# djene-mengistu/UAPS

Hardware: AMD Instinct MI355X
Metric: training images/sec (labeled+unlabeled) NEU-Seg 256x256 K=3 (higher is better)
Workload: dtype f32

## Files before the change

### uaps_amd/csrc/conv_split_wrw.hpp

```cpp
#pragma once
#include "conv_split.hpp"

namespace uaps {

#ifndef UAPS_WRW_ABLATE
#define UAPS_WRW_ABLATE 0
#endif

template <int TH, int WCO, int WCI, int DIL = 1> struct SWrwCfg {
    static constexpr int TW = 32, WR = 4 / (WCO * WCI), RPW = TH / WR;
    static constexpr int BCO = 16 * WCO, BCI = 16 * WCI;
    static constexpr int XG = DIL > 1 ? 6 : 4;
    static constexpr int DPLU = TH * 4 + 2;
    static constexpr int XPLU = (TH + 2) * XG + 2;
    static constexpr int EPL = (TH + 2) * 4 + 1;
    static constexpr int ND = (BCO * TH * 4 + kConvThreads - 1) / kConvThreads;
    static constexpr int NX = (BCI * (TH + 2) * XG + kConvThreads - 1) / kConvThreads;
    static_assert(WCO * WCI * WR == 4 && TH % WR == 0, "wave arrangement");
};

__device__ __forceinline__ void split8(const float (&v)[8], u32x4& p0, u32x4& p1, u32x4& p2) {
#pragma unroll
    for (int i = 0; i < 4; ++i) {
        unsigned a, b, c;
        conv_split3(v[2 * i], v[2 * i + 1], a, b, c);
        p0[i] = a; p1[i] = b; p2[i] = c;
    }
}

__device__ __forceinline__ void split8h(const float (&v)[8], float sc, u32x4& p0, u32x4& p1) {
    const f32x2 sc2 = bcast_lo(sc);
#pragma unroll
    for (int i = 0; i < 4; ++i) {
        const f32x2 t = f32x2{v[2 * i], v[2 * i + 1]} * sc2;
        unsigned a, b;
        conv_split2h(t.x, t.y, a, b);
        p0[i] = a; p1[i] = b;
    }
}

template <int TH, int WCO, int WCI, bool XF, bool H16 = false, int DIL = 1>
__device__ __forceinline__ void conv_swrw_body(const ConvWrwArgs& a) {
    using Cfg = SWrwCfg<TH, WCO, WCI, DIL>;
    static_assert(DIL == 1 || ((DIL == 2 || DIL == 4) && H16 && !XF), "dilated form: fp16 pieces, no staging-time BatchNorm");
    constexpr int NP = H16 ? 2 : 3;
    constexpr int XG = Cfg::XG, XH = DIL > 1 ? 1 : 0;
    constexpr int TW = 32, WR = Cfg::WR, RPW = Cfg::RPW, BCO = Cfg::BCO, BCI = Cfg::BCI;
    constexpr int DPLU = Cfg::DPLU, XPLU = Cfg::XPLU, EPL = Cfg::EPL, ND = Cfg::ND, NX = Cfg::NX;
    constexpr int RED_FLOATS = WR > 1 ? (WR / 2) * WCO * WCI * 10 * 256 : 0;
    constexpr bool EU = H16 && DIL == 1;
    constexpr int XGS = EU ? 5 : XG;
    constexpr int XPLS = EU ? (TH + 2) * 5 + ((TH + 2) * 5 % 4 == 2 ? 0 : (6 - (TH + 2) * 5 % 4) % 4) : XPLU;
    static_assert(XPLS % 4 == 2, "input plane stride");
    constexpr int NE = EU ? (BCI * (TH + 2) + kConvThreads - 1) / kConvThreads : 0;
    constexpr int STAGE_UNITS = NP * BCO * DPLU + NP * BCI * XPLS;
    constexpr int LDS_UNITS = STAGE_UNITS > RED_FLOATS / 4 ? STAGE_UNITS : RED_FLOATS / 4;

    __shared__ __attribute__((aligned(16))) u32x4 smem[LDS_UNITS];
    __shared__ unsigned sE[(DIL == 1 && !EU) ? NP * BCI * EPL : 1];
    __shared__ f32x2 sXf[XF ? kWrwMaxGroups * BCI + 1 : 1];
    u32x4* sD = smem;
    u32x4* sX = smem + NP * BCO * DPLU;
    constexpr int XF_ZERO = kWrwMaxGroups * BCI;

    float sc_d = 1.f, sc_x = 1.f, inv_d = 1.f, inv_x = 1.f;
    if constexpr (H16) {
        const f32x2 sd = h16_scale(bound_of(a.dy_bound, a.dy_mul));
        const f32x2 sx = h16_scale(__builtin_fmaxf(bound_of(a.in_bound, a.in_mul), bound_of(a.in2_bound, a.in2_mul)));
        sc_d = sd.x; inv_d = sd.y; sc_x = sx.x; inv_x = sx.y;
    }

    const int tid = threadIdx.x, lane = tid & 63, wave = tid >> 6;
    const int j = lane & 15, kq = lane >> 4;
    const int wr = wave % WR, wci = (wave / WR) % WCI, wco = wave / (WR * WCI);

    int bid = xcd_swizzle(blockIdx.x, gridDim.x);
    if (bid >= a.nsplit * a.ncob * a.ncib) return;
    stagger_by_wave_slot();
    const int cib = bid % a.ncib; bid /= a.ncib;
    const int cob = bid % a.ncob;
    const int split = bid / a.ncob;
    const int co0 = cob * BCO, ci0 = cib * BCI;
    const int HW = a.H * a.W;
    const int tiles_per_img = a.tiles_x * a.tiles_y, ntiles = a.B * tiles_per_img;
    const int t_begin = (int)((long)ntiles * split / a.nsplit), t_end = (int)((long)ntiles * (split + 1) / a.nsplit);
    const bool want_bias = a.bslab != nullptr && cib == 0;

    int dC[ND], dR[ND], dG[ND];
    int xC[NX], xR[NX], xG[NX];
#pragma unroll
    for (int n = 0; n < ND; ++n) {
        const int u = tid + n * kConvThreads;
        dC[n] = u < BCO * TH * 4 ? u / (TH * 4) : -1; dR[n] = (u / 4) % TH; dG[n] = u % 4;
    }
#pragma unroll
    for (int n = 0; n < NX; ++n) {
        const int u = tid + n * kConvThreads;
        xC[n] = u < BCI * (TH + 2) * XG ? u / ((TH + 2) * XG) : -1; xR[n] = (u / XG) % (TH + 2); xG[n] = u % XG;
    }
    if constexpr (XF) {
        const int G = a.B / a.xf_Bg;
        for (int i = tid; i < G * BCI; i += kConvThreads) {
            const int g = i / BCI, ch = ci0 + i % BCI;
            f32x2 v = f32x2{0.f, 0.f};
            if (ch < a.Cin) { const float2 t = a.xf[(size_t)g * a.Cin + ch]; v = f32x2{t.x, t.y}; }
            sXf[i] = v;
        }
        if (tid == 0) sXf[XF_ZERO] = f32x2{0.f, 0.f};
    }

    float rd[ND][8];
    float rx[NX][(DIL == 1 && !EU) ? 10 : 8];
    float re[EU ? NE : 1][2];
    int eC[EU ? NE : 1], eR[EU ? NE : 1];
    if constexpr (EU) {
#pragma unroll
        for (int n = 0; n < NE; ++n) {
            const int i = tid + n * kConvThreads;
            eC[n] = i < BCI * (TH + 2) ? i / (TH + 2) : -1; eR[n] = i % (TH + 2);
        }
    }
    int xf_idx[XF ? NX : 1];
    int exf_idx[(XF && EU) ? NE : 1];

    auto load_tile = [&](int t) {
        const int b = t / tiles_per_img, tt = t % tiles_per_img;
        const int ry = a.col_major ? tt % a.tiles_y : tt / a.tiles_x, x0 = (a.col_major ? tt / a.tiles_y : tt % a.tiles_x) * TW;
        const int y0 = DIL == 1 ? ry * TH : ry % DIL + (ry / DIL) * (TH * DIL);
#pragma unroll
        for (int n = 0; n < ND; ++n) {
            const int c = co0 + dC[n], gy = y0 + dR[n] * DIL, gx = x0 + dG[n] * 8;
#if UAPS_WRW_ABLATE & 4
            {
                const int cc = c < 0 ? 0 : (c < a.Cout ? c : a.Cout - 1), yy = gy < a.H ? gy : a.H - 1, xx = gx + 8 <= a.W ? gx : a.W - 8;
                const float* q = a.dout + ((size_t)b * a.Cout + cc) * HW + yy * a.W + xx;
                const f32x4 w0 = *reinterpret_cast<const f32x4*>(q), w1 = *reinterpret_cast<const f32x4*>(q + 4);
#pragma unroll
                for (int k = 0; k < 4; ++k) { rd[n][k] = w0[k]; rd[n][4 + k] = w1[k]; }
                continue;
            }
#endif
            const bool ok = dC[n] >= 0 && c < a.Cout && gy < a.H && gx < a.W;
            const float* p = a.dout + ((size_t)b * a.Cout + (ok ? c : 0)) * HW + (ok ? gy * a.W + gx : 0);
            const f32x4 v0 = ok ? *reinterpret_cast<const f32x4*>(p) : f32x4{0.f, 0.f, 0.f, 0.f};
            const f32x4 v1 = (ok && gx + 4 < a.W) ? *reinterpret_cast<const f32x4*>(p + 4) : f32x4{0.f, 0.f, 0.f, 0.f};
#pragma unroll
            for (int k = 0; k < 4; ++k) { rd[n][k] = v0[k]; rd[n][4 + k] = v1[k]; }
        }
#pragma unroll
        for (int n = 0; n < NX; ++n) {
            const int c = ci0 + xC[n], gy = y0 + (xR[n] - 1) * DIL, gx = x0 + (xG[n] - XH) * 8;
#if UAPS_WRW_ABLATE & 8
            if (xR[n] == 0 || xR[n] == TH + 1) continue;
#endif
#if UAPS_WRW_ABLATE & 4
            {
                const int cc = c < 0 ? 0 : (c < a.Csplit ? c : a.Csplit - 1), yy = gy < 0 ? 0 : (gy < a.H ? gy : a.H - 1);
                const int xx = gx < 0 ? 0 : (gx + 8 <= a.W ? gx : a.W - 8);
                const float* q = a.in + ((size_t)b * a.Csplit + cc) * HW + yy * a.W;
                const f32x4 w0 = *reinterpret_cast<const f32x4*>(q + xx), w1 = *reinterpret_cast<const f32x4*>(q + xx + 4);
#pragma unroll
                for (int k = 0; k < 4; ++k) { rx[n][k] = w0[k]; rx[n][4 + k] = w1[k]; }
                if constexpr (DIL == 1 && !EU) {
#if !(UAPS_WRW_ABLATE & 2)
                    rx[n][8] = q[xx > 0 ? xx - 1 : 0]; rx[n][9] = q[xx + 8 < a.W ? xx + 8 : a.W - 1];
#else
                    rx[n][8] = 0.f; rx[n][9] = 0.f;
#endif
                }
                if constexpr (XF) xf_idx[n] = (b / a.xf_Bg) * BCI + (xC[n] < 0 ? 0 : xC[n]);
                continue;
            }
#endif
            const bool second = c >= a.Csplit;
            const float* src = second ? a.in2 + ((size_t)b * (a.Cin - a.Csplit) + (c - a.Csplit)) * HW : a.in + ((size_t)b * a.Csplit + c) * HW;
            const bool okc = xC[n] >= 0 && c < a.Cin && gy >= 0 && gy < a.H;
            const bool ok = okc && gx >= 0 && gx < a.W;
            const float* p = src + (okc ? gy * a.W : 0) + (ok ? gx : 0);
            const f32x4 v0 = ok ? *reinterpret_cast<const f32x4*>(p) : f32x4{0.f, 0.f, 0.f, 0.f};
            const f32x4 v1 = (ok && gx + 4 < a.W) ? *reinterpret_cast<const f32x4*>(p + 4) : f32x4{0.f, 0.f, 0.f, 0.f};
#pragma unroll
            for (int k = 0; k < 4; ++k) { rx[n][k] = v0[k]; rx[n][4 + k] = v1[k]; }
            if constexpr (DIL == 1 && !EU) {
#if UAPS_WRW_ABLATE & 2
                rx[n][8] = 0.f; rx[n][9] = 0.f;
#else
                rx[n][8] = (okc && gx - 1 >= 0 && gx - 1 < a.W) ? src[gy * a.W + gx - 1] : 0.f;
                rx[n][9] = (okc && gx + 8 < a.W) ? src[gy * a.W + gx + 8] : 0.f;
#endif
            }
            if constexpr (XF) xf_idx[n] = okc ? (b / a.xf_Bg) * BCI + xC[n] : XF_ZERO;
        }
        if constexpr (EU) {
#pragma unroll
            for (int n = 0; n < NE; ++n) {
                const int c = ci0 + eC[n], gy = y0 + eR[n] - 1;
                const bool second = c >= a.Csplit;
                const float* src = second ? a.in2 + ((size_t)b * (a.Cin - a.Csplit) + (c - a.Csplit)) * HW : a.in + ((size_t)b * a.Csplit + c) * HW;
                const bool okc = eC[n] >= 0 && c < a.Cin && gy >= 0 && gy < a.H;
#if UAPS_WRW_ABLATE & 2
                re[n][0] = 0.f; re[n][1] = 0.f;
#else
                re[n][0] = (okc && x0 - 1 >= 0) ? src[gy * a.W + x0 - 1] : 0.f;
                re[n][1] = (okc && x0 + TW < a.W) ? src[gy * a.W + x0 + TW] : 0.f;
#endif
                if constexpr (XF) exf_idx[n] = okc ? (b / a.xf_Bg) * BCI + eC[n] : XF_ZERO;
            }
        }
    };
    auto store_tile = [&](int t) {
        const int tt = t % tiles_per_img;
        const int x0 = (a.col_major ? tt / a.tiles_y : tt % a.tiles_x) * TW;
#pragma unroll
        for (int n = 0; n < ND; ++n) {
            if (dC[n] < 0) continue;
            const int u = dC[n] * DPLU + dR[n] * 4 + dG[n];
            if constexpr (H16) {
                u32x4 p0, p1;
                split8h(rd[n], sc_d, p0, p1);
                sD[u] = p0; sD[BCO * DPLU + u] = p1;
            } else {
                u32x4 p0, p1, p2;
                split8(rd[n], p0, p1, p2);
                sD[u] = p0; sD[BCO * DPLU + u] = p1; sD[2 * BCO * DPLU + u] = p2;
            }
        }
#pragma unroll
        for (int n = 0; n < NX; ++n) {
            if (xC[n] < 0) continue;
#if UAPS_WRW_ABLATE & 8
            if (xR[n] == 0 || xR[n] == TH + 1) continue;
#endif
            if constexpr (XF) {
                const f32x2 cf = sXf[xf_idx[n]];
                const int gx = x0 + xG[n] * 8;
#pragma unroll
                for (int k = 0; k < ((DIL == 1 && !EU) ? 10 : 8); ++k) {
                    const int col = k < 8 ? gx + k : (k == 8 ? gx - 1 : gx + 8);
                    const float z = __builtin_fmaf(rx[n][k], cf.x, cf.y);
                    rx[n][k] = (col >= 0 && col < a.W) ? __builtin_fmaxf(z, z * a.xf_slope) : 0.f;
                }
            }
            float v8[8];
#pragma unroll
            for (int k = 0; k < 8; ++k) v8[k] = rx[n][k];
            const int u = xC[n] * XPLS + xR[n] * XGS + xG[n];
            const int eu = xC[n] * EPL + xR[n] * 4 + xG[n];
            if constexpr (DIL > 1) {
                u32x4 p0, p1;
                split8h(v8, sc_x, p0, p1);
                sX[u] = p0; sX[BCI * XPLS + u] = p1;
            } else if constexpr (EU) {
                u32x4 p0, p1;
                split8h(v8, sc_x, p0, p1);
                sX[u] = p0; sX[BCI * XPLS + u] = p1;
                (void)eu;
            } else if constexpr (H16) {
                u32x4 p0, p1;
                split8h(v8, sc_x, p0, p1);
                sX[u] = p0; sX[BCI * XPLS + u] = p1;
#if !(UAPS_WRW_ABLATE & 2)
                unsigned e0, e1;
                const f32x2 ev = f32x2{rx[n][9], rx[n][8]} * bcast_lo(sc_x);
                conv_split2h(ev.x, ev.y, e0, e1);
                sE[eu] = e0; sE[BCI * EPL + eu] = e1;
#else
                (void)eu;
#endif
            } else {
                u32x4 p0, p1, p2;
                split8(v8, p0, p1, p2);
                sX[u] = p0; sX[BCI * XPLS + u] = p1; sX[2 * BCI * XPLS + u] = p2;
                unsigned e0, e1, e2;
                conv_split3(rx[n][9], rx[n][8], e0, e1, e2);
                sE[eu] = e0; sE[BCI * EPL + eu] = e1; sE[2 * BCI * EPL + eu] = e2;
            }
        }
        if constexpr (EU) {
#if !(UAPS_WRW_ABLATE & 2)
#pragma unroll
            for (int n = 0; n < NE; ++n) {
                if (eC[n] < 0) continue;
                float l = re[n][0], r = re[n][1];
                if constexpr (XF) {
                    const f32x2 cf = sXf[exf_idx[n]];
                    const float zl = __builtin_fmaf(l, cf.x, cf.y), zr = __builtin_fmaf(r, cf.x, cf.y);
                    l = x0 - 1 >= 0 ? __builtin_fmaxf(zl, zl * a.xf_slope) : 0.f;
                    r = x0 + TW < a.W ? __builtin_fmaxf(zr, zr * a.xf_slope) : 0.f;
                }
                unsigned e0, e1;
                const f32x2 ev = f32x2{r, l} * bcast_lo(sc_x);
                conv_split2h(ev.x, ev.y, e0, e1);
                const int ue = eC[n] * XPLS + eR[n] * XGS + 4;
                sX[ue] = u32x4{e0, e0, e0, e0}; sX[BCI * XPLS + ue] = u32x4{e1, e1, e1, e1};
            }
#endif
        }
    };

    f32x4 acc[9];
    f32x4 accb = f32x4{0.f, 0.f, 0.f, 0.f};
#pragma unroll
    for (int t = 0; t < 9; ++t) acc[t] = f32x4{0.f, 0.f, 0.f, 0.f};
    constexpr unsigned kOnes = H16 ? 0x3C003C00u : 0x3F803F80u;
    const u32x4 ones_u = u32x4{kOnes, kOnes, kOnes, kOnes};
    const bf16x8 ones = __builtin_bit_cast(bf16x8, ones_u);

    const int aoff = (wco * 16 + j) * DPLU + kq;
    const int boff = (wci * 16 + j) * XPLS + kq + XH;
    const int eoff = (wci * 16 + j) * EPL + kq;
    const int elidx = ((kq + 4) % 5) * 4 + 3, eridx = (kq + 1) * 4;

    if (t_begin < t_end) { load_tile(t_begin); }
    if constexpr (XF) __syncthreads();
    if (t_begin < t_end) store_tile(t_begin);
    __syncthreads();
    for (int t = t_begin; t < t_end; ++t) {
        const bool more = t + 1 < t_end;
        if (more) load_tile(t + 1);
#pragma unroll
        for (int rr = 0; rr < RPW + 2; ++rr) {
            const int r = wr * RPW + rr;
            bf16x8 bf[3][NP];
#pragma unroll
            for (int p = 0; p < NP; ++p) {
                const u32x4 c = sX[p * BCI * XPLS + boff + r * XGS];
                if constexpr (DIL > 1) {
                    const unsigned* cl = reinterpret_cast<const unsigned*>(&sX[p * BCI * XPLS + boff + r * XGS - 1]);
                    const unsigned* cr = reinterpret_cast<const unsigned*>(&sX[p * BCI * XPLS + boff + r * XGS + 1]);
                    if constexpr (DIL == 2) {
                        bf[0][p] = __builtin_bit_cast(bf16x8, u32x4{cl[3], c[0], c[1], c[2]});
                        bf[2][p] = __builtin_bit_cast(bf16x8, u32x4{c[1], c[2], c[3], cr[0]});
                    } else {
                        bf[0][p] = __builtin_bit_cast(bf16x8, u32x4{cl[2], cl[3], c[0], c[1]});
                        bf[2][p] = __builtin_bit_cast(bf16x8, u32x4{c[2], c[3], cr[0], cr[1]});
                    }
                    bf[1][p] = __builtin_bit_cast(bf16x8, c);
                    continue;
                }
#if UAPS_WRW_ABLATE & 1
                bf[0][p] = __builtin_bit_cast(bf16x8, c); bf[1][p] = __builtin_bit_cast(bf16x8, c); bf[2][p] = __builtin_bit_cast(bf16x8, c);
                continue;
#endif
                unsigned el, er;
#if UAPS_WRW_ABLATE & 2
                el = er = 0u;
#else
                if constexpr (EU) {
                    const unsigned* rowd = reinterpret_cast<const unsigned*>(&sX[p * BCI * XPLS + (wci * 16 + j) * XPLS + r * XGS]);
                    el = rowd[elidx]; er = rowd[eridx];
                } else {
                    el = er = sE[p * BCI * EPL + eoff + r * 4];
                }
#endif
                const unsigned t01 = __builtin_amdgcn_alignbit(c[1], c[0], 16), t12 = __builtin_amdgcn_alignbit(c[2], c[1], 16);
                const unsigned t23 = __builtin_amdgcn_alignbit(c[3], c[2], 16);
                const unsigned tE0 = __builtin_amdgcn_alignbit(c[0], el, 16), t3E = __builtin_amdgcn_alignbit(er, c[3], 16);
                bf[0][p] = __builtin_bit_cast(bf16x8, u32x4{tE0, t01, t12, t23});
                bf[1][p] = __builtin_bit_cast(bf16x8, c);
                bf[2][p] = __builtin_bit_cast(bf16x8, u32x4{t01, t12, t23, t3E});
            }
#pragma unroll
            for (int ky = 0; ky < 3; ++ky) {
                const int yy = rr - ky;
                if (yy < 0 || yy >= RPW) continue;
                bf16x8 af[NP];
#pragma unroll
                for (int p = 0; p < NP; ++p) af[p] = __builtin_bit_cast(bf16x8, sD[p * BCO * DPLU + aoff + (wr * RPW + yy) * 4]);
#pragma unroll
                for (int kx = 0; kx < 3; ++kx) {
                    f32x4 c = acc[ky * 3 + kx];
                    if constexpr (H16) {
                        const auto H = [](const bf16x8& v) { return __builtin_bit_cast(f16x8, v); };
                        c = __builtin_amdgcn_mfma_f32_16x16x32_f16(H(af[1]), H(bf[kx][0]), c, 0, 0, 0);
                        c = __builtin_amdgcn_mfma_f32_16x16x32_f16(H(af[0]), H(bf[kx][1]), c, 0, 0, 0);
                        c = __builtin_amdgcn_mfma_f32_16x16x32_f16(H(af[0]), H(bf[kx][0]), c, 0, 0, 0);
                    } else {
                    c = __builtin_amdgcn_mfma_f32_16x16x32_bf16(af[2], bf[kx][0], c, 0, 0, 0);
                    c = __builtin_amdgcn_mfma_f32_16x16x32_bf16(af[0], bf[kx][2], c, 0, 0, 0);
                    c = __builtin_amdgcn_mfma_f32_16x16x32_bf16(af[1], bf[kx][1], c, 0, 0, 0);
                    c = __builtin_amdgcn_mfma_f32_16x16x32_bf16(af[1], bf[kx][0], c, 0, 0, 0);
                    c = __builtin_amdgcn_mfma_f32_16x16x32_bf16(af[0], bf[kx][1], c, 0, 0, 0);
                    c = __builtin_amdgcn_mfma_f32_16x16x32_bf16(af[0], bf[kx][0], c, 0, 0, 0);
                    }
                    acc[ky * 3 + kx] = c;
                }
                if (ky == 0 && want_bias && wci == 0) {
                    if constexpr (H16) {
                        accb = __builtin_amdgcn_mfma_f32_16x16x32_f16(__builtin_bit_cast(f16x8, af[1]), __builtin_bit_cast(f16x8, ones), accb, 0, 0, 0);
                        accb = __builtin_amdgcn_mfma_f32_16x16x32_f16(__builtin_bit_cast(f16x8, af[0]), __builtin_bit_cast(f16x8, ones), accb, 0, 0, 0);
                    } else {
                        accb = __builtin_amdgcn_mfma_f32_16x16x32_bf16(af[2], ones, accb, 0, 0, 0);
                        accb = __builtin_amdgcn_mfma_f32_16x16x32_bf16(af[1], ones, accb, 0, 0, 0);
                        accb = __builtin_amdgcn_mfma_f32_16x16x32_bf16(af[0], ones, accb, 0, 0, 0);
                    }
                }
            }
        }
        __syncthreads();
        if (more) store_tile(t + 1);
        __syncthreads();
    }

    if constexpr (WR > 1) {
        float* red = reinterpret_cast<float*>(smem);
#pragma unroll
        for (int s = WR / 2; s >= 1; s >>= 1) {
            if (wr >= s && wr < 2 * s) {
                float* p = red + (size_t)(((wr - s) * WCO + wco) * WCI + wci) * 10 * 256 + lane;
#pragma unroll
                for (int t = 0; t < 9; ++t)
#pragma unroll
                    for (int r = 0; r < 4; ++r) p[(t * 4 + r) * 64] = acc[t][r];
#pragma unroll
                for (int r = 0; r < 4; ++r) p[(36 + r) * 64] = accb[r];
            }
            __syncthreads();
            if (wr < s) {
                const float* p = red + (size_t)((wr * WCO + wco) * WCI + wci) * 10 * 256 + lane;
#pragma unroll
                for (int t = 0; t < 9; ++t)
#pragma unroll
                    for (int r = 0; r < 4; ++r) acc[t][r] += p[(t * 4 + r) * 64];
#pragma unroll
                for (int r = 0; r < 4; ++r) accb[r] += p[(36 + r) * 64];
            }
            __syncthreads();
        }
    }
    if (wr != 0) return;
    float* slab = a.slab + (size_t)split * 9 * a.CoutS * a.CinS;
    float chk = 0.f;
    const f32x2 id2 = bcast_lo(inv_d), ix2 = bcast_lo(inv_x);
#pragma unroll
    for (int t = 0; t < 9; ++t) {
        if constexpr (H16) note_nonfinite(chk, acc[t]);
#pragma unroll
        for (int r = 0; r < 4; r += 2) {
            f32x2 v = f32x2{acc[t][r], acc[t][r + 1]};
            if constexpr (H16) v = (v * id2) * ix2;
            const int co = co0 + wco * 16 + kq * 4 + r, ci = ci0 + wci * 16 + j;
            slab[((size_t)t * a.CoutS + co) * a.CinS + ci] = v.x;
            slab[((size_t)t * a.CoutS + co + 1) * a.CinS + ci] = v.y;
        }
    }
    if constexpr (H16) report_nonfinite(a.err, chk, UAPS_ERR_WRW_NONFINITE);
    if (want_bias && wci == 0 && j == 0) {
#pragma unroll
        for (int r = 0; r < 4; r += 2) {
            f32x2 v = f32x2{accb[r], accb[r + 1]};
            if constexpr (H16) v = v * id2;
            a.bslab[(size_t)split * a.CoutS + co0 + wco * 16 + kq * 4 + r] = v.x;
            a.bslab[(size_t)split * a.CoutS + co0 + wco * 16 + kq * 4 + r + 1] = v.y;
        }
    }
}

template <int TH, int WCO, int WCI>
__global__ __launch_bounds__(kConvThreads, 2) void conv_swrw_kernel(ConvWrwArgs a) { conv_swrw_body<TH, WCO, WCI, false>(a); }
template <int TH, int WCO, int WCI>
__global__ __launch_bounds__(kConvThreads, 2) void conv_swrw_bn_kernel(ConvWrwArgs a) { conv_swrw_body<TH, WCO, WCI, true>(a); }
template <int TH, int WCO, int WCI>
__global__ __launch_bounds__(kConvThreads, 2) void conv_hwrw_kernel(ConvWrwArgs a) { conv_swrw_body<TH, WCO, WCI, false, true>(a); }
template <int TH, int WCO, int WCI>
__global__ __launch_bounds__(kConvThreads, 2) void conv_hwrw_bn_kernel(ConvWrwArgs a) { conv_swrw_body<TH, WCO, WCI, true, true>(a); }
template <int TH, int WCO, int WCI, int DIL>
__global__ __launch_bounds__(kConvThreads, 2) void conv_hwrw_d_kernel(ConvWrwArgs a) { conv_swrw_body<TH, WCO, WCI, false, true, DIL>(a); }

}
```

Before: 2682.

## Restage weight-gradient input tile in transposed LDS layout read via ds_read_tr16

The weight-gradient conv kernel now stages input activations as channel-interleaved rows: each thread loads 8 channels by 4 pixels. The rows are stored in a swizzled column-slot LDS layout that already includes the halo columns, so the separate edge buffer and alignbit shifting are no longer needed. B fragments are read with the ds_read_tr16_b64 transpose instruction and double-buffered across rows. Bias accumulation moves out of the inner loop. The aim is fewer LDS shuffles and ALU ops per MFMA, at the cost of more global loads per thread (strided across channels), more registers, and removal of the ablation switches.

```diff
diff --git a/uaps_amd/csrc/conv_split_wrw.hpp b/uaps_amd/csrc/conv_split_wrw.hpp
--- a/uaps_amd/csrc/conv_split_wrw.hpp
+++ b/uaps_amd/csrc/conv_split_wrw.hpp
@@ -2,22 +2,30 @@
 #include "conv_split.hpp"
 
 namespace uaps {
-
-#ifndef UAPS_WRW_ABLATE
-#define UAPS_WRW_ABLATE 0
-#endif
 
 template <int TH, int WCO, int WCI, int DIL = 1> struct SWrwCfg {
     static constexpr int TW = 32, WR = 4 / (WCO * WCI), RPW = TH / WR;
     static constexpr int BCO = 16 * WCO, BCI = 16 * WCI;
-    static constexpr int XG = DIL > 1 ? 6 : 4;
     static constexpr int DPLU = TH * 4 + 2;
-    static constexpr int XPLU = (TH + 2) * XG + 2;
-    static constexpr int EPL = (TH + 2) * 4 + 1;
     static constexpr int ND = (BCO * TH * 4 + kConvThreads - 1) / kConvThreads;
-    static constexpr int NX = (BCI * (TH + 2) * XG + kConvThreads - 1) / kConvThreads;
+    static constexpr int NCB = BCI / 16, NR = NCB * (TH + 2);
+    static constexpr int XS = TW + 2 * DIL;
+    static constexpr int XRB = 32 * (XS + 1);
+    static constexpr int XPB = NR * XRB;
+    static constexpr int NXU = 2 * ((NR + 3) / 4 * 4) * 10;
+    static constexpr int NX = (NXU + kConvThreads - 1) / kConvThreads;
     static_assert(WCO * WCI * WR == 4 && TH % WR == 0, "wave arrangement");
+    static_assert(XS % 2 == 0 && XRB % 128 != 0 && XRB % 64 == 32 && XS <= 40, "input row stride");
 };
+
+__device__ __forceinline__ constexpr int swrw_slot(int s) { return s ^ (((s >> 3) & 1) << 2); }
+
+typedef short s16x4 __attribute__((ext_vector_type(4)));
+typedef __attribute__((address_space(3))) s16x4 lds_s16x4;
+
+__device__ __forceinline__ s16x4 swrw_read_tr(const char* p) {
+    return __builtin_amdgcn_ds_read_tr16_b64_v4i16((lds_s16x4*)p);
+}
 
 __device__ __forceinline__ void split8(const float (&v)[8], u32x4& p0, u32x4& p1, u32x4& p2) {
 #pragma unroll
@@ -44,23 +52,18 @@
     using Cfg = SWrwCfg<TH, WCO, WCI, DIL>;
     static_assert(DIL == 1 || ((DIL == 2 || DIL == 4) && H16 && !XF), "dilated form: fp16 pieces, no staging-time BatchNorm");
     constexpr int NP = H16 ? 2 : 3;
-    constexpr int XG = Cfg::XG, XH = DIL > 1 ? 1 : 0;
     constexpr int TW = 32, WR = Cfg::WR, RPW = Cfg::RPW, BCO = Cfg::BCO, BCI = Cfg::BCI;
-    constexpr int DPLU = Cfg::DPLU, XPLU = Cfg::XPLU, EPL = Cfg::EPL, ND = Cfg::ND, NX = Cfg::NX;
+    constexpr int DPLU = Cfg::DPLU, ND = Cfg::ND, NX = Cfg::NX;
+    constexpr int NR = Cfg::NR, XS = Cfg::XS, XRB = Cfg::XRB, XPB = Cfg::XPB;
     constexpr int RED_FLOATS = WR > 1 ? (WR / 2) * WCO * WCI * 10 * 256 : 0;
-    constexpr bool EU = H16 && DIL == 1;
-    constexpr int XGS = EU ? 5 : XG;
-    constexpr int XPLS = EU ? (TH + 2) * 5 + ((TH + 2) * 5 % 4 == 2 ? 0 : (6 - (TH + 2) * 5 % 4) % 4) : XPLU;
-    static_assert(XPLS % 4 == 2, "input plane stride");
-    constexpr int NE = EU ? (BCI * (TH + 2) + kConvThreads - 1) / kConvThreads : 0;
-    constexpr int STAGE_UNITS = NP * BCO * DPLU + NP * BCI * XPLS;
+    constexpr int STAGE_UNITS = NP * BCO * DPLU + NP * XPB / 16;
     constexpr int LDS_UNITS = STAGE_UNITS > RED_FLOATS / 4 ? STAGE_UNITS : RED_FLOATS / 4;
+    static_assert(XPB % 16 == 0, "input plane alignment");
 
     __shared__ __attribute__((aligned(16))) u32x4 smem[LDS_UNITS];
-    __shared__ unsigned sE[(DIL == 1 && !EU) ? NP * BCI * EPL : 1];
     __shared__ f32x2 sXf[XF ? kWrwMaxGroups * BCI + 1 : 1];
     u32x4* sD = smem;
-    u32x4* sX = smem + NP * BCO * DPLU;
+    char* sX = reinterpret_cast<char*>(smem + NP * BCO * DPLU);
     constexpr int XF_ZERO = kWrwMaxGroups * BCI;
 
     float sc_d = 1.f, sc_x = 1.f, inv_d = 1.f, inv_x = 1.f;
@@ -87,7 +90,7 @@
     const bool want_bias = a.bslab != nullptr && cib == 0;
 
     int dC[ND], dR[ND], dG[ND];
-    int xC[NX], xR[NX], xG[NX];
+    int xR[NX], xQ[NX], xH[NX];
 #pragma unroll
     for (int n = 0; n < ND; ++n) {
         const int u = tid + n * kConvThreads;
@@ -95,8 +98,9 @@
     }
 #pragma unroll
     for (int n = 0; n < NX; ++n) {
-        const int u = tid + n * kConvThreads;
-        xC[n] = u < BCI * (TH + 2) * XG ? u / ((TH + 2) * XG) : -1; xR[n] = (u / XG) % (TH + 2); xG[n] = u % XG;
+        const int u = tid + n * kConvThreads, w = u >> 3;
+        const int R = 4 * (w / 10) + ((u >> 1) & 3);
+        xR[n] = u < Cfg::NXU && R < NR ? R : -1; xQ[n] = w % 10; xH[n] = u & 1;
     }
     if constexpr (XF) {
         const int G = a.B / a.xf_Bg;
@@ -110,18 +114,9 @@
     }
 
     float rd[ND][8];
-    float rx[NX][(DIL == 1 && !EU) ? 10 : 8];
-    float re[EU ? NE : 1][2];
-    int eC[EU ? NE : 1], eR[EU ? NE : 1];
-    if constexpr (EU) {
-#pragma unroll
-        for (int n = 0; n < NE; ++n) {
-            const int i = tid + n * kConvThreads;
-            eC[n] = i < BCI * (TH + 2) ? i / (TH + 2) : -1; eR[n] = i % (TH + 2);
-        }
-    }
+    float rx[NX][8][4];
+    bool xok[NX];
     int xf_idx[XF ? NX : 1];
-    int exf_idx[(XF && EU) ? NE : 1];
 
     auto load_tile = [&](int t) {
         const int b = t / tiles_per_img, tt = t % tiles_per_img;
@@ -130,16 +125,6 @@
 #pragma unroll
         for (int n = 0; n < ND; ++n) {
             const int c = co0 + dC[n], gy = y0 + dR[n] * DIL, gx = x0 + dG[n] * 8;
-#if UAPS_WRW_ABLATE & 4
-            {
-                const int cc = c < 0 ? 0 : (c < a.Cout ? c : a.Cout - 1), yy = gy < a.H ? gy : a.H - 1, xx = gx + 8 <= a.W ? gx : a.W - 8;
-                const float* q = a.dout + ((size_t)b * a.Cout + cc) * HW + yy * a.W + xx;
-                const f32x4 w0 = *reinterpret_cast<const f32x4*>(q), w1 = *reinterpret_cast<const f32x4*>(q + 4);
-#pragma unroll
-                for (int k = 0; k < 4; ++k) { rd[n][k] = w0[k]; rd[n][4 + k] = w1[k]; }
-                continue;
-            }
-#endif
             const bool ok = dC[n] >= 0 && c < a.Cout && gy < a.H && gx < a.W;
             const float* p = a.dout + ((size_t)b * a.Cout + (ok ? c : 0)) * HW + (ok ? gy * a.W + gx : 0);
             const f32x4 v0 = ok ? *reinterpret_cast<const f32x4*>(p) : f32x4{0.f, 0.f, 0.f, 0.f};
@@ -149,68 +134,25 @@
         }
 #pragma unroll
         for (int n = 0; n < NX; ++n) {
-            const int c = ci0 + xC[n], gy = y0 + (xR[n] - 1) * DIL, gx = x0 + (xG[n] - XH) * 8;
-#if UAPS_WRW_ABLATE & 8
-            if (xR[n] == 0 || xR[n] == TH + 1) continue;
-#endif
-#if UAPS_WRW_ABLATE & 4
-            {
-                const int cc = c < 0 ? 0 : (c < a.Csplit ? c : a.Csplit - 1), yy = gy < 0 ? 0 : (gy < a.H ? gy : a.H - 1);
-                const int xx = gx < 0 ? 0 : (gx + 8 <= a.W ? gx : a.W - 8);
-                const float* q = a.in + ((size_t)b * a.Csplit + cc) * HW + yy * a.W;
-                const f32x4 w0 = *reinterpret_cast<const f32x4*>(q + xx), w1 = *reinterpret_cast<const f32x4*>(q + xx + 4);
-#pragma unroll
-                for (int k = 0; k < 4; ++k) { rx[n][k] = w0[k]; rx[n][4 + k] = w1[k]; }
-                if constexpr (DIL == 1 && !EU) {
-#if !(UAPS_WRW_ABLATE & 2)
-                    rx[n][8] = q[xx > 0 ? xx - 1 : 0]; rx[n][9] = q[xx + 8 < a.W ? xx + 8 : a.W - 1];
-#else
-                    rx[n][8] = 0.f; rx[n][9] = 0.f;
-#endif
-                }
-                if constexpr (XF) xf_idx[n] = (b / a.xf_Bg) * BCI + (xC[n] < 0 ? 0 : xC[n]);
-                continue;
-            }
-#endif
+            const int R = xR[n] < 0 ? 0 : xR[n], cb = R / (TH + 2), r = R % (TH + 2);
+            const int c = ci0 + cb * 16 + xH[n] * 8, gy = y0 + (r - 1) * DIL, gx = x0 + xQ[n] * 4 - 4;
             const bool second = c >= a.Csplit;
             const float* src = second ? a.in2 + ((size_t)b * (a.Cin - a.Csplit) + (c - a.Csplit)) * HW : a.in + ((size_t)b * a.Csplit + c) * HW;
-            const bool okc = xC[n] >= 0 && c < a.Cin && gy >= 0 && gy < a.H;
-            const bool ok = okc && gx >= 0 && gx < a.W;
-            const float* p = src + (okc ? gy * a.W : 0) + (ok ? gx : 0);
-            const f32x4 v0 = ok ? *reinterpret_cast<const f32x4*>(p) : f32x4{0.f, 0.f, 0.f, 0.f};
-            const f32x4 v1 = (ok && gx + 4 < a.W) ? *reinterpret_cast<const f32x4*>(p + 4) : f32x4{0.f, 0.f, 0.f, 0.f};
-#pragma unroll
-            for (int k = 0; k < 4; ++k) { rx[n][k] = v0[k]; rx[n][4 + k] = v1[k]; }
-            if constexpr (DIL == 1 && !EU) {
-#if UAPS_WRW_ABLATE & 2
-                rx[n][8] = 0.f; rx[n][9] = 0.f;
-#else
-                rx[n][8] = (okc && gx - 1 >= 0 && gx - 1 < a.W) ? src[gy * a.W + gx - 1] : 0.f;
-                rx[n][9] = (okc && gx + 8 < a.W) ? src[gy * a.W + gx + 8] : 0.f;
-#endif
-            }
-            if constexpr (XF) xf_idx[n] = okc ? (b / a.xf_Bg) * BCI + xC[n] : XF_ZERO;
-        }
-        if constexpr (EU) {
-#pragma unroll
-            for (int n = 0; n < NE; ++n) {
-                const int c = ci0 + eC[n], gy = y0 + eR[n] - 1;
-                const bool second = c >= a.Csplit;
-                const float* src = second ? a.in2 + ((size_t)b * (a.Cin - a.Csplit) + (c - a.Csplit)) * HW : a.in + ((size_t)b * a.Csplit + c) * HW;
-                const bool okc = eC[n] >= 0 && c < a.Cin && gy >= 0 && gy < a.H;
-#if UAPS_WRW_ABLATE & 2
-                re[n][0] = 0.f; re[n][1] = 0.f;
-#else
-                re[n][0] = (okc && x0 - 1 >= 0) ? src[gy * a.W + x0 - 1] : 0.f;
-                re[n][1] = (okc && x0 + TW < a.W) ? src[gy * a.W + x0 + TW] : 0.f;
-#endif
-                if constexpr (XF) exf_idx[n] = okc ? (b / a.xf_Bg) * BCI + eC[n] : XF_ZERO;
-            }
+            const bool okr = xR[n] >= 0 && gy >= 0 && gy < a.H;
+            const bool ok = okr && gx >= 0 && gx < a.W;
+            const float* p = src + (ok ? gy * a.W + gx : 0);
+#pragma unroll
+            for (int i = 0; i < 8; ++i) {
+                const f32x4 v = (ok && c + i < a.Cin) ? *reinterpret_cast<const f32x4*>(p + (size_t)i * HW) : f32x4{0.f, 0.f, 0.f, 0.f};
+#pragma unroll
+                for (int k = 0; k < 4; ++k) rx[n][i][k] = v[k];
+            }
+            xok[n] = ok;
+            if constexpr (XF) xf_idx[n] = (b / a.xf_Bg) * BCI + cb * 16 + xH[n] * 8;
         }
     };
     auto store_tile = [&](int t) {
-        const int tt = t % tiles_per_img;
-        const int x0 = (a.col_major ? tt / a.tiles_y : tt % a.tiles_x) * TW;
+        (void)t;
 #pragma unroll
         for (int n = 0; n < ND; ++n) {
             if (dC[n] < 0) continue;
@@ -227,74 +169,37 @@
         }
 #pragma unroll
         for (int n = 0; n < NX; ++n) {
-            if (xC[n] < 0) continue;
-#if UAPS_WRW_ABLATE & 8
-            if (xR[n] == 0 || xR[n] == TH + 1) continue;
-#endif
+            if (xR[n] < 0) continue;
             if constexpr (XF) {
-                const f32x2 cf = sXf[xf_idx[n]];
-                const int gx = x0 + xG[n] * 8;
-#pragma unroll
-                for (int k = 0; k < ((DIL == 1 && !EU) ? 10 : 8); ++k) {
-                    const int col = k < 8 ? gx + k : (k == 8 ? gx - 1 : gx + 8);
-                    const float z = __builtin_fmaf(rx[n][k], cf.x, cf.y);
-                    rx[n][k] = (col >= 0 && col < a.W) ? __builtin_fmaxf(z, z * a.xf_slope) : 0.f;
-                }
-            }
-            float v8[8];
-#pragma unroll
-            for (int k = 0; k < 8; ++k) v8[k] = rx[n][k];
-            const int u = xC[n] * XPLS + xR[n] * XGS + xG[n];
-            const int eu = xC[n] * EPL + xR[n] * 4 + xG[n];
-            if constexpr (DIL > 1) {
-                u32x4 p0, p1;
-                split8h(v8, sc_x, p0, p1);
-                sX[u] = p0; sX[BCI * XPLS + u] = p1;
-            } else if constexpr (EU) {
-                u32x4 p0, p1;
-                split8h(v8, sc_x, p0, p1);
-                sX[u] = p0; sX[BCI * XPLS + u] = p1;
-                (void)eu;
-            } else if constexpr (H16) {
-                u32x4 p0, p1;
-                split8h(v8, sc_x, p0, p1);
-                sX[u] = p0; sX[BCI * XPLS + u] = p1;
-#if !(UAPS_WRW_ABLATE & 2)
-                unsigned e0, e1;
-                const f32x2 ev = f32x2{rx[n][9], rx[n][8]} * bcast_lo(sc_x);
-                conv_split2h(ev.x, ev.y, e0, e1);
-                sE[eu] = e0; sE[BCI * EPL + eu] = e1;
-#else
-                (void)eu;
-#endif
-            } else {
-                u32x4 p0, p1, p2;
-                split8(v8, p0, p1, p2);
-                sX[u] = p0; sX[BCI * XPLS + u] = p1; sX[2 * BCI * XPLS + u] = p2;
-                unsigned e0, e1, e2;
-                conv_split3(rx[n][9], rx[n][8], e0, e1, e2);
-                sE[eu] = e0; sE[BCI * EPL + eu] = e1; sE[2 * BCI * EPL + eu] = e2;
-            }
-        }
-        if constexpr (EU) {
-#if !(UAPS_WRW_ABLATE & 2)
-#pragma unroll
-            for (int n = 0; n < NE; ++n) {
-                if (eC[n] < 0) continue;
-                float l = re[n][0], r = re[n][1];
-                if constexpr (XF) {
-                    const f32x2 cf = sXf[exf_idx[n]];
-                    const float zl = __builtin_fmaf(l, cf.x, cf.y), zr = __builtin_fmaf(r, cf.x, cf.y);
-                    l = x0 - 1 >= 0 ? __builtin_fmaxf(zl, zl * a.xf_slope) : 0.f;
-                    r = x0 + TW < a.W ? __builtin_fmaxf(zr, zr * a.xf_slope) : 0.f;
-                }
-                unsigned e0, e1;
-                const f32x2 ev = f32x2{r, l} * bcast_lo(sc_x);
-                conv_split2h(ev.x, ev.y, e0, e1);
-                const int ue = eC[n] * XPLS + eR[n] * XGS + 4;
-                sX[ue] = u32x4{e0, e0, e0, e0}; sX[BCI * XPLS + ue] = u32x4{e1, e1, e1, e1};
-            }
-#endif
+#pragma unroll
+                for (int i = 0; i < 8; ++i) {
+                    const f32x2 cf = sXf[xf_idx[n] + i];
+#pragma unroll
+                    for (int k = 0; k < 4; ++k) {
+                        const float z = __builtin_fmaf(rx[n][i][k], cf.x, cf.y);
+                        rx[n][i][k] = xok[n] ? __builtin_fmaxf(z, z * a.xf_slope) : 0.f;
+                    }
+                }
+            }
+            char* row = sX + xR[n] * XRB + xH[n] * 16;
+#pragma unroll
+            for (int k = 0; k < 4; ++k) {
+                const int s = xQ[n] * 4 - 4 + k + DIL;
+                if (DIL < 4 && (s < 0 || s >= XS)) continue;
+                float v8[8];
+#pragma unroll
+                for (int i = 0; i < 8; ++i) v8[i] = rx[n][i][k];
+                u32x4* q = reinterpret_cast<u32x4*>(row + swrw_slot(s) * 32);
+                if constexpr (H16) {
+                    u32x4 p0, p1;
+                    split8h(v8, sc_x, p0, p1);
+                    q[0] = p0; q[XPB / 16] = p1;
+                } else {
+                    u32x4 p0, p1, p2;
+                    split8(v8, p0, p1, p2);
+                    q[0] = p0; q[XPB / 16] = p1; q[2 * XPB / 16] = p2;
+                }
+            }
         }
     };
 
@@ -307,9 +212,12 @@
     const bf16x8 ones = __builtin_bit_cast(bf16x8, ones_u);
 
     const int aoff = (wco * 16 + j) * DPLU + kq;
-    const int boff = (wci * 16 + j) * XPLS + kq + XH;
-    const int eoff = (wci * 16 + j) * EPL + kq;
-    const int elidx = ((kq + 4) % 5) * 4 + 3, eridx = (kq + 1) * 4;
+    int xo[3][2];
+#pragma unroll
+    for (int kx = 0; kx < 3; ++kx)
+#pragma unroll
+        for (int h = 0; h < 2; ++h)
+            xo[kx][h] = (wci * (TH + 2) + wr * RPW) * XRB + swrw_slot(8 * kq + kx * DIL + 4 * h + (j >> 2)) * 32 + (j & 3) * 8;
 
     if (t_begin < t_end) { load_tile(t_begin); }
     if constexpr (XF) __syncthreads();
@@ -318,48 +226,22 @@
     for (int t = t_begin; t < t_end; ++t) {
         const bool more = t + 1 < t_end;
         if (more) load_tile(t + 1);
+        bf16x8 bf[2][3][NP];
+        auto read_b = [&](int rr, bf16x8 (&f)[3][NP]) {
+#pragma unroll
+            for (int p = 0; p < NP; ++p)
+#pragma unroll
+                for (int kx = 0; kx < 3; ++kx) {
+                    const char* base = sX + p * XPB + rr * XRB;
+                    const s16x4 lo = swrw_read_tr(base + xo[kx][0]), hi = swrw_read_tr(base + xo[kx][1]);
+                    f[kx][p] = __builtin_bit_cast(bf16x8, __builtin_shufflevector(lo, hi, 0, 1, 2, 3, 4, 5, 6, 7));
+                }
+        };
+        read_b(0, bf[0]);
 #pragma unroll
         for (int rr = 0; rr < RPW + 2; ++rr) {
-            const int r = wr * RPW + rr;
-            bf16x8 bf[3][NP];
-#pragma unroll
-            for (int p = 0; p < NP; ++p) {
-                const u32x4 c = sX[p * BCI * XPLS + boff + r * XGS];
-                if constexpr (DIL > 1) {
-                    const unsigned* cl = reinterpret_cast<const unsigned*>(&sX[p * BCI * XPLS + boff + r * XGS - 1]);
-                    const unsigned* cr = reinterpret_cast<const unsigned*>(&sX[p * BCI * XPLS + boff + r * XGS + 1]);
-                    if constexpr (DIL == 2) {
-                        bf[0][p] = __builtin_bit_cast(bf16x8, u32x4{cl[3], c[0], c[1], c[2]});
-                        bf[2][p] = __builtin_bit_cast(bf16x8, u32x4{c[1], c[2], c[3], cr[0]});
-                    } else {
-                        bf[0][p] = __builtin_bit_cast(bf16x8, u32x4{cl[2], cl[3], c[0], c[1]});
-                        bf[2][p] = __builtin_bit_cast(bf16x8, u32x4{c[2], c[3], cr[0], cr[1]});
-                    }
-                    bf[1][p] = __builtin_bit_cast(bf16x8, c);
-                    continue;
-                }
-#if UAPS_WRW_ABLATE & 1
-                bf[0][p] = __builtin_bit_cast(bf16x8, c); bf[1][p] = __builtin_bit_cast(bf16x8, c); bf[2][p] = __builtin_bit_cast(bf16x8, c);
-                continue;
-#endif
-                unsigned el, er;
-#if UAPS_WRW_ABLATE & 2
-                el = er = 0u;
-#else
-                if constexpr (EU) {
-                    const unsigned* rowd = reinterpret_cast<const unsigned*>(&sX[p * BCI * XPLS + (wci * 16 + j) * XPLS + r * XGS]);
-                    el = rowd[elidx]; er = rowd[eridx];
-                } else {
-                    el = er = sE[p * BCI * EPL + eoff + r * 4];
-                }
-#endif
-                const unsigned t01 = __builtin_amdgcn_alignbit(c[1], c[0], 16), t12 = __builtin_amdgcn_alignbit(c[2], c[1], 16);
-                const unsigned t23 = __builtin_amdgcn_alignbit(c[3], c[2], 16);
-                const unsigned tE0 = __builtin_amdgcn_alignbit(c[0], el, 16), t3E = __builtin_amdgcn_alignbit(er, c[3], 16);
-                bf[0][p] = __builtin_bit_cast(bf16x8, u32x4{tE0, t01, t12, t23});
-                bf[1][p] = __builtin_bit_cast(bf16x8, c);
-                bf[2][p] = __builtin_bit_cast(bf16x8, u32x4{t01, t12, t23, t3E});
-            }
+            if (rr + 1 < RPW + 2) read_b(rr + 1, bf[(rr + 1) & 1]);
+            const bf16x8 (&b)[3][NP] = bf[rr & 1];
 #pragma unroll
             for (int ky = 0; ky < 3; ++ky) {
                 const int yy = rr - ky;
@@ -372,28 +254,34 @@
                     f32x4 c = acc[ky * 3 + kx];
                     if constexpr (H16) {
                         const auto H = [](const bf16x8& v) { return __builtin_bit_cast(f16x8, v); };
-                        c = __builtin_amdgcn_mfma_f32_16x16x32_f16(H(af[1]), H(bf[kx][0]), c, 0, 0, 0);
-                        c = __builtin_amdgcn_mfma_f32_16x16x32_f16(H(af[0]), H(bf[kx][1]), c, 0, 0, 0);
-                        c = __builtin_amdgcn_mfma_f32_16x16x32_f16(H(af[0]), H(bf[kx][0]), c, 0, 0, 0);
+                        c = __builtin_amdgcn_mfma_f32_16x16x32_f16(H(af[1]), H(b[kx][0]), c, 0, 0, 0);
+                        c = __builtin_amdgcn_mfma_f32_16x16x32_f16(H(af[0]), H(b[kx][1]), c, 0, 0, 0);
+                        c = __builtin_amdgcn_mfma_f32_16x16x32_f16(H(af[0]), H(b[kx][0]), c, 0, 0, 0);
                     } else {
-                    c = __builtin_amdgcn_mfma_f32_16x16x32_bf16(af[2], bf[kx][0], c, 0, 0, 0);
-                    c = __builtin_amdgcn_mfma_f32_16x16x32_bf16(af[0], bf[kx][2], c, 0, 0, 0);
-                    c = __builtin_amdgcn_mfma_f32_16x16x32_bf16(af[1], bf[kx][1], c, 0, 0, 0);
-                    c = __builtin_amdgcn_mfma_f32_16x16x32_bf16(af[1], bf[kx][0], c, 0, 0, 0);
-                    c = __builtin_amdgcn_mfma_f32_16x16x32_bf16(af[0], bf[kx][1], c, 0, 0, 0);
-                    c = __builtin_amdgcn_mfma_f32_16x16x32_bf16(af[0], bf[kx][0], c, 0, 0, 0);
+                    c = __builtin_amdgcn_mfma_f32_16x16x32_bf16(af[2], b[kx][0], c, 0, 0, 0);
+                    c = __builtin_amdgcn_mfma_f32_16x16x32_bf16(af[0], b[kx][2], c, 0, 0, 0);
+                    c = __builtin_amdgcn_mfma_f32_16x16x32_bf16(af[1], b[kx][1], c, 0, 0, 0);
+                    c = __builtin_amdgcn_mfma_f32_16x16x32_bf16(af[1], b[kx][0], c, 0, 0, 0);
+                    c = __builtin_amdgcn_mfma_f32_16x16x32_bf16(af[0], b[kx][1], c, 0, 0, 0);
+                    c = __builtin_amdgcn_mfma_f32_16x16x32_bf16(af[0], b[kx][0], c, 0, 0, 0);
                     }
                     acc[ky * 3 + kx] = c;
                 }
-                if (ky == 0 && want_bias && wci == 0) {
-                    if constexpr (H16) {
-                        accb = __builtin_amdgcn_mfma_f32_16x16x32_f16(__builtin_bit_cast(f16x8, af[1]), __builtin_bit_cast(f16x8, ones), accb, 0, 0, 0);
-                        accb = __builtin_amdgcn_mfma_f32_16x16x32_f16(__builtin_bit_cast(f16x8, af[0]), __builtin_bit_cast(f16x8, ones), accb, 0, 0, 0);
-                    } else {
-                        accb = __builtin_amdgcn_mfma_f32_16x16x32_bf16(af[2], ones, accb, 0, 0, 0);
-                        accb = __builtin_amdgcn_mfma_f32_16x16x32_bf16(af[1], ones, accb, 0, 0, 0);
-                        accb = __builtin_amdgcn_mfma_f32_16x16x32_bf16(af[0], ones, accb, 0, 0, 0);
-                    }
+            }
+        }
+        if (want_bias && wci == 0) {
+#pragma unroll
+            for (int yy = 0; yy < RPW; ++yy) {
+                bf16x8 af[NP];
+#pragma unroll
+                for (int p = 0; p < NP; ++p) af[p] = __builtin_bit_cast(bf16x8, sD[p * BCO * DPLU + aoff + (wr * RPW + yy) * 4]);
+                if constexpr (H16) {
+                    accb = __builtin_amdgcn_mfma_f32_16x16x32_f16(__builtin_bit_cast(f16x8, af[1]), __builtin_bit_cast(f16x8, ones), accb, 0, 0, 0);
+                    accb = __builtin_amdgcn_mfma_f32_16x16x32_f16(__builtin_bit_cast(f16x8, af[0]), __builtin_bit_cast(f16x8, ones), accb, 0, 0, 0);
+                } else {
+                    accb = __builtin_amdgcn_mfma_f32_16x16x32_bf16(af[2], ones, accb, 0, 0, 0);
+                    accb = __builtin_amdgcn_mfma_f32_16x16x32_bf16(af[1], ones, accb, 0, 0, 0);
+                    accb = __builtin_amdgcn_mfma_f32_16x16x32_bf16(af[0], ones, accb, 0, 0, 0);
                 }
             }
         }
```

After: 2696, median of 6. Within noise of the previous version (+0.5%).
